# simplify23/MRN

Hardware: AMD Instinct MI355X
Metric: text-line images/sec (fwd+bwd) at 32x256, TRBA+MRN 6 experts (higher is better)
Workload: dtype f32; 1 GPU; MRN loop B: TRBAx6 frozen experts fwd + DM-Router fwd/bwd + clip + Adam, 32x256x4 crops; per_gpu_batch=256, global_batch=256, parallelism=dp1

## Files before the change

mrn_amd/_lib.py:

```python
import ctypes
import os
import re

import torch

_HERE = os.path.dirname(os.path.abspath(__file__))
LIB_PATH = os.environ.get("MRN_LIB_PATH") or os.path.join(_HERE, "csrc", "libmrn_hip.so")
HEADER_PATH = os.path.join(os.path.dirname(_HERE), "include", "mrn_hip.h")
DECODE_HEADER_PATH = os.path.join(os.path.dirname(_HERE), "include", "mrn_decode.h")
ATTN_BEAM_HEADER_PATH = os.path.join(os.path.dirname(_HERE), "include", "mrn_attn_beam.h")
LEXICON_HEADER_PATH = os.path.join(os.path.dirname(_HERE), "include", "mrn_lexicon.h")

_CTYPES = {
    "int": ctypes.c_int,
    "int64_t": ctypes.c_int64,
    "float": ctypes.c_float,
    "void*": ctypes.c_void_p,
    "float*": ctypes.c_void_p,
    "const float*": ctypes.c_void_p,
    "const int64_t*": ctypes.c_void_p,
    "int64_t*": ctypes.c_void_p,
    "const int*": ctypes.c_void_p,
    "int*": ctypes.c_void_p,
    "const int32_t*": ctypes.c_void_p,
    "int32_t*": ctypes.c_void_p,
    "const void*": ctypes.c_void_p,
# ... 24 lines not shown


class _Lib:
    def __init__(self):
        self._dll = None
        self._protos = None

    def load(self):
        if self._dll is not None:
            return self._dll
        if not os.path.exists(LIB_PATH):
            raise RuntimeError(
                f"{LIB_PATH} is missing: build it with `python -m mrn_amd.build` (there is no CPU fallback)")
        dll = ctypes.CDLL(LIB_PATH)
        self._protos = {**parse_header(), **parse_header(DECODE_HEADER_PATH), **parse_header(ATTN_BEAM_HEADER_PATH),
                        **parse_header(LEXICON_HEADER_PATH)}
        for name, (ret, argtypes, _) in self._protos.items():
            fn = getattr(dll, name)
            fn.restype = _CTYPES[ret]
            fn.argtypes = [_CTYPES[t] for t in argtypes]
        self._dll = dll
        return dll

    def call(self, name, *args):
        dll = self.load()
        fn = getattr(dll, name)
        rc = fn(*args)
        if fn.restype is ctypes.c_int and rc != 0:
            msg = dll.mrn_last_error().decode()
            raise RuntimeError(f"{name} failed (code {rc}): {msg}")
        return rc
# ... 8 lines not shown
```

mrn_amd/csrc/common.hpp:

```cpp
#pragma once
#include <hip/hip_runtime.h>
#include <stdint.h>
#include <stdio.h>
#include <string.h>

#define MRN_EXPORT extern "C" __attribute__((visibility("default")))

enum {
  MRN_OK = 0,
  MRN_ERR_BAD_ARG = -1,
  MRN_ERR_UNSUPPORTED = -2,
  MRN_ERR_WORKSPACE = -3,
};

void mrn_set_error(const char* fmt, ...);

#define MRN_CHECK_ARG(cond, ...)          \
  do {                                    \
    if (!(cond)) {                        \
      mrn_set_error(__VA_ARGS__);         \
      return MRN_ERR_BAD_ARG;             \
    }                                     \
  } while (0)

// ... 19 lines not shown
  int base = (xcd < r) ? xcd * (q + 1) : r * (q + 1) + (xcd - r) * q;
  return base + idx;
}

__device__ __forceinline__ void split_f16(float x, _Float16& hi, _Float16& lo) {
  asm volatile("" : "+v"(x));
  hi = (_Float16)x;
  lo = (_Float16)(x - (float)hi);
}

__device__ __forceinline__ void split_f16_sat(float x, _Float16& hi, _Float16& lo) {
  x = fminf(fmaxf(x, -65504.f), 65504.f);
  split_f16(x, hi, lo);
}

__device__ __forceinline__ float relu_nan(float v, float floor_ = 0.f) { return v != v ? v : fmaxf(v, floor_); }
__device__ __forceinline__ float max_nan(float a, float b) { return (a != a || b != b) ? a + b : fmaxf(a, b); }

__device__ __forceinline__ float gelu_fast(float x) {
  const float z = fabsf(x) * 0.70710678118654752440f;
  const float t = __builtin_amdgcn_rcpf(fmaf(0.3275911f, z, 1.f));
  float pl = fmaf(1.061405429f, t, -1.453152027f);
  pl = fmaf(pl, t, 1.421413741f);
  pl = fmaf(pl, t, -0.284496736f);
  pl = fmaf(pl, t, 0.254829592f);
  const float e = pl * t * __builtin_amdgcn_exp2f(-z * z * 1.4426950408889634f);
  const float cdf = x >= 0.f ? fmaf(-0.5f, e, 1.f) : 0.5f * e;
  return x * cdf;
}

// ... 38 lines not shown
```

mrn_amd/csrc/conv_patch.hip:

```cpp
#include "common.hpp"
#include <stdlib.h>

namespace {

typedef _Float16 f16v8 __attribute__((ext_vector_type(8)));
typedef unsigned u32x4 __attribute__((ext_vector_type(4)));
typedef __attribute__((address_space(3))) void* lds_ptr_t;

struct ConvPatchParams {
  const unsigned char* x;
  const unsigned char* w;
  const float* w_scale;
  const float* bias;
  const long long* gamma;
  float* y;
  float* stats;
  long x_gstride;
  int x_bytes;
  int B, H, W, act, pool;
  int tiles_x, tiles_y, tiles;
  int rows;
};

template <int CB, int NCO, int NST>
struct Cfg {
  static constexpr int RG = 4 / NCO;
  static constexpr int TH = 4 * RG, TW = 32;
  static constexpr int PR = TH + 2, PC = TW + 2;
  static constexpr int NL = CB * PR * PC;
  static constexpr int NDMA = (NL + 7) / 8;
  static constexpr int NJ = (NDMA + 3) / 4;
  static constexpr int STAGE = NJ * 4 * 1024;
  static constexpr bool LEAN = CB == 2;
  static constexpr int STATS = LEAN ? 4 * 8 * 64 * 16 : 0;
  static constexpr int LDS = NST * STAGE + STATS;
  static constexpr int NS = CB * 9 * 2;
};

__device__ __forceinline__ f32x16 mma(const u32x4 a, const u32x4 b, const f32x16 c) {
#ifdef MRN_PPROBE_NO_MFMA
  f32x16 r = c;
  r[0] += __builtin_bit_cast(float, a[0] ^ b[0]);
  return r;
#endif
  return __builtin_amdgcn_mfma_f32_32x32x16_f16(*reinterpret_cast<const f16v8*>(&a), *reinterpret_cast<const f16v8*>(&b), c, 0, 0, 0);
}

#ifdef MRN_PPROBE_TIMING
__device__ unsigned long long g_patch_dbg[8];
extern "C" __attribute__((visibility("default"))) int mrn_patch_dbg_read(unsigned long long* out, int reset) {
  if (hipMemcpyFromSymbol(out, HIP_SYMBOL(g_patch_dbg), sizeof(g_patch_dbg)) != hipSuccess) return -1;
  if (reset) {
// ... 1 lines not shown
    (void)hipMemcpyToSymbol(HIP_SYMBOL(g_patch_dbg), z, sizeof(z));
  }
  return 0;
}
#define PTICK(var) const long var = __builtin_readcyclecounter()
#define PADD(slot, a, b) dbg_acc[slot] += (b) - (a)
#else
#define PTICK(var)
#define PADD(slot, a, b)
#endif

__device__ __forceinline__ float swap1(float v) {
  return __builtin_bit_cast(float, __builtin_amdgcn_mov_dpp(__builtin_bit_cast(int, v), 0xB1, 0xF, 0xF, true));
}

template <int CB, int NCO, int NST, bool POOL, int NPROD = 3>
__global__ __launch_bounds__(256) void conv_patch_x3_kernel(const ConvPatchParams p) {
  using C = Cfg<CB, NCO, NST>;
  constexpr int PR = C::PR, PC = C::PC, TH = C::TH, STAGE = C::STAGE;
  extern __shared__ __attribute__((aligned(1024))) unsigned char lds[];
  const int t = threadIdx.x, lane = t & 63, wave = __builtin_amdgcn_readfirstlane(t >> 6);
  const int n = lane & 31, kh = lane >> 5;
  const int g = blockIdx.y;
  const int cob = wave % NCO, rg = wave / NCO;
  const int co0 = cob * 32;
  constexpr int Cout = NCO * 32;

  u32x4 Wh[CB][9][2], Wl[CB][9][2];
  {
    const unsigned char* wg = p.w + ((long)g * Cout + co0 + n) * (CB * 9 * 128) + kh * 16;
#pragma unroll
// ... 36 lines not shown
    a.x0 = (r2 - ty * p.tiles_x) * C::TW;
    a.base = (((a.b * p.H + a.y0 - 1) * p.W + a.x0 - 1) * CB) * 128;
    return a;
  };
  auto issue_dma = [&](int i, const TileAt& a, int stage, bool live) {
    const int L = 8 * (wave + 4 * i) + (lane >> 3);
    const int cb = CB == 1 ? 0 : (L >= PR * PC ? 1 : 0), rem = L - cb * (PR * PC);
    const int prow = (rem * 1928) >> 16, pcol = rem - prow * PC;
    static_assert(PC == 34 && C::NJ * 32 < 1024, "the division by the patch width is a multiply-shift");
    const int y = a.y0 - 1 + prow, x = a.x0 - 1 + pcol;
    const bool ok = live && L < C::NL && (unsigned)y < (unsigned)p.H && (unsigned)x < (unsigned)p.W;
    const int rel = ((prow * p.W + pcol) * CB + cb) * 128 + (((lane & 7) ^ ((pcol >> 1) & 7)) << 4);
    const int okm = -(int)ok;
    const int voff = ((a.base + rel) & okm) | ((int)0x80000000 & ~okm);
    __builtin_amdgcn_raw_ptr_buffer_load_lds(xr, (lds_ptr_t)(lds + stage * STAGE + (wave + 4 * i) * 1024), 16, voff, 0, 0, 0);
  };

  constexpr int RP = 2, NPASS = 4 / RP;
  f32x16 accA[RP], accB[RP];
#pragma unroll
  for (int r = 0; r < RP; ++r)
#pragma unroll
    for (int e = 0; e < 16; ++e) accA[r][e] = accB[r][e] = 0.f;
  f32x4 hold = {0.f, 0.f, 0.f, 0.f};
  struct Pending { int off, ok0, ok1, okp, live; };
  Pending pend = {0, 0, 0, 0, 0};
  constexpr bool LEAN = C::LEAN, PIPE = !LEAN;
  f32x4 st_s[LEAN ? 1 : 4], st_q[LEAN ? 1 : 4];
  f32x4 bias4[LEAN ? 1 : 4];
  unsigned char* const st_base = lds + NST * STAGE + (wave * 8 * 64 + lane) * 16;
// ... 111 lines not shown
      }
      if (LEAN) *reinterpret_cast<f32x4*>(st_base + c * 1024) = f32x4{0.f, 0.f, 0.f, 0.f};
      else if (c < 4) st_s[LEAN ? 0 : c] = f32x4{0.f, 0.f, 0.f, 0.f};
      else st_q[LEAN ? 0 : c - 4] = f32x4{0.f, 0.f, 0.f, 0.f};
    }
    if (n == 0 && p.stats) {
      float* dst = p.stats + (((long)g * p.rows + row) * C::RG + rg) * 2 * Cout + co0 + 4 * kh;
#pragma unroll
      for (int c = 0; c < 8; ++c) *reinterpret_cast<f32x4*>(dst + (c >> 2) * Cout + 8 * (c & 3)) = v[c];
    }
  };
  int row = blockIdx.x, tile = row, stage = 0;
  int flush_row = -1;
  TileAt cur = locate(tile < p.tiles ? tile : 0);
  if (tile < p.tiles) {
#pragma unroll
    for (int i = 0; i < C::NJ; ++i) issue_dma(i, cur, 0, true);
  }
  __builtin_amdgcn_s_waitcnt((7 << 4) | (15 << 8));
#ifdef MRN_PPROBE_TIMING
  long dbg_acc[6] = {0, 0, 0, 0, 0, 0};
#endif
  while (tile < p.tiles) {
    PTICK(tk0);
    asm volatile("s_waitcnt lgkmcnt(0)" ::: "memory");
    __builtin_amdgcn_s_barrier();
    asm volatile("" ::: "memory");
    PTICK(tk1);
    PADD(0, tk0, tk1);
    int nxt = tile + p.rows, nrow = row;
    if (nxt >= p.tiles) {
      nrow = row + gridDim.x;
// ... 16 lines not shown
#pragma unroll
        for (int r = 0; r < RP; ++r) {
          const int imm = (cb * PR + ps * RP + r + dy) * PC * 128;
          if constexpr (NPROD == 3) Xl[set][r] = *reinterpret_cast<const u32x4*>(lds + offv[dx][1][ks] + imm);
          Xh[set][r] = *reinterpret_cast<const u32x4*>(lds + offv[dx][0][ks] + imm);
        }
      };
      PTICK(tm0);
      read_X(0, 0);
      constexpr int DMA_PER_STEP = (C::NJ + C::NS - 3) / (C::NS - 2);
      constexpr int EPI0 = 1;
#pragma unroll
      for (int s = 0; s < C::NS; ++s) {
        const int cb = s / 18, tap = (s % 18) >> 1, ks = s & 1, set = s & 1;
        if (s + 1 < C::NS) read_X(s + 1, set ^ 1);
        if (ps == 0) {
#pragma unroll
          for (int i = s * DMA_PER_STEP; i < (s + 1) * DMA_PER_STEP; ++i)
            if (i < C::NJ) issue_dma(i, nx, stage ^ 1, more);
        }
        if (PIPE && s >= EPI0 && s < EPI0 + 8) epilogue_slice(accp, s - EPI0);
        if constexpr (NPROD == 3) {
#pragma unroll
          for (int r = 0; r < RP; ++r) acc[r] = mma(Wh[cb][tap][ks], Xl[set][r], acc[r]);
#pragma unroll
          for (int r = 0; r < RP; ++r) acc[r] = mma(Wl[cb][tap][ks], Xh[set][r], acc[r]);
        }
#pragma unroll
        for (int r = 0; r < RP; ++r) acc[r] = mma(Wh[cb][tap][ks], Xh[set][r], acc[r]);
#define PATCH_SGB(mask, n) __builtin_amdgcn_sched_group_barrier(mask, n, 0);
#define PATCH_INTERLEAVE PATCH_SGB(0x008, 1) PATCH_SGB(0x002, 6) PATCH_SGB(0x100, 1) PATCH_SGB(0x020, 1) PATCH_SGB(0x040, 1)
        PATCH_INTERLEAVE PATCH_INTERLEAVE
        if constexpr (NPROD == 3) { PATCH_INTERLEAVE PATCH_INTERLEAVE PATCH_INTERLEAVE PATCH_INTERLEAVE }
        __builtin_amdgcn_sched_barrier(0);
      }
      if (ps == 0 && flush_row >= 0) {
        flush_stats(flush_row);
        flush_row = -1;
      }
      pend = make_pending(cur, ps);
      if (!PIPE) {
#pragma unroll
        for (int j = 0; j < 8; ++j) epilogue_slice(acc, j);
        pend.live = 0;
      }
      PTICK(tm1);
      PADD(1, tm0, tm1);
      if (ps == NPASS - 1) __builtin_amdgcn_s_waitcnt((7 << 4) | (15 << 8));
// ... 47 lines not shown

}

MRN_EXPORT int64_t mrn_conv3x3_patch_supported(int Cin, int Cout) { return (Cin == 32 && Cout == 64) || (Cin == 64 && Cout == 128); }

static int patch_rows(long tiles) { return (int)(tiles < 1008 ? tiles : 1008); }

MRN_EXPORT int64_t mrn_conv3x3_patch_stats_blocks(int G, int B, int H, int W, int Cin) {
  (void)G;
  const int TH = Cin == 32 ? 8 : 4, RG = Cin == 32 ? 2 : 1;
  return (int64_t)patch_rows((long)B * ((H + TH - 1) / TH) * ((W + 31) / 32)) * RG;
}

static int patch_launch(const void* x_hl, const void* w_hl, const float* w_scale, const float* bias,
                        const void* bn_gamma_ptrs, float* y, float* stats, int G, int64_t x_group_stride_bytes, int B,
                        int H, int W, int Cin, int Cout, int act, int pool, int products, void* stream) {
  MRN_CHECK_ARG(x_hl && w_hl && w_scale && y && G >= 1 && mrn_conv3x3_patch_supported(Cin, Cout),
                "mrn_conv3x3_patch_x3_hl32: bad operands (Cin=%d Cout=%d)", Cin, Cout);
  MRN_CHECK_ARG(!pool || (H % 2 == 0 && W % 2 == 0), "mrn_conv3x3_patch_x3_hl32: the pooled form needs even H, W (%d x %d)", H, W);
  MRN_CHECK_ARG((long)B * H * W * Cin * 4 < 2147483647L && (long)B * H * W * Cout * 4 < 2147483647L && (uintptr_t)x_hl % 16 == 0 &&
                    (uintptr_t)w_hl % 16 == 0 && (uintptr_t)y % 16 == 0,
                "mrn_conv3x3_patch_x3_hl32: one expert's input and output must stay below 2 GiB each and be 16-byte aligned");
  if (B == 0 || H == 0 || W == 0) return MRN_OK;
  ConvPatchParams p;
  p.x = (const unsigned char*)x_hl; p.w = (const unsigned char*)w_hl; p.w_scale = w_scale; p.bias = bias;
  p.gamma = (const long long*)bn_gamma_ptrs; p.y = y; p.stats = stats; p.x_gstride = x_group_stride_bytes;
  p.x_bytes = (int)((long)B * H * W * Cin * 4);
  p.B = B; p.H = H; p.W = W; p.act = act; p.pool = pool;
  const int TH = Cin == 32 ? 8 : 4;
  p.tiles_x = (W + 31) / 32; p.tiles_y = (H + TH - 1) / TH; p.tiles = B * p.tiles_x * p.tiles_y;
  p.rows = patch_rows(p.tiles);
  int wgs = patch_wgs(G, p.tiles, 1);
  if (wgs > p.rows) wgs = p.rows;
#define PATCH_LAUNCH(CB_, NCO_, POOL_, NP_)                                                                                              \
  do {                                                                                                                                   \
    using C = Cfg<CB_, NCO_, 2>;                                                                                                          \
    static bool set = false;                                                                                                             \
    if (!set) {                                                                                                                          \
      (void)hipFuncSetAttribute((const void*)conv_patch_x3_kernel<CB_, NCO_, 2, POOL_, NP_>, hipFuncAttributeMaxDynamicSharedMemorySize, C::LDS); \
      set = true;                                                                                                                        \
    }                                                                                                                                    \
    hipLaunchKernelGGL((conv_patch_x3_kernel<CB_, NCO_, 2, POOL_, NP_>), dim3(wgs, G), dim3(256), C::LDS, (hipStream_t)stream, p);      \
  } while (0)
#define PATCH_LAUNCH_P(CB_, NCO_, POOL_) do { if (products == 1) PATCH_LAUNCH(CB_, NCO_, POOL_, 1); else PATCH_LAUNCH(CB_, NCO_, POOL_, 3); } while (0)
  if (Cin == 32) {
    if (pool) PATCH_LAUNCH_P(1, 2, true);
    else PATCH_LAUNCH_P(1, 2, false);
  } else {
    if (pool) PATCH_LAUNCH_P(2, 4, true);
    else PATCH_LAUNCH_P(2, 4, false);
  }
#undef PATCH_LAUNCH_P
#undef PATCH_LAUNCH
  MRN_LAUNCH_CHECK("conv3x3_patch_x3");
  return MRN_OK;
}

MRN_EXPORT int mrn_conv3x3_patch_x3_hl32(const void* x_hl, const void* w_hl, const float* w_scale, const float* bias,
                                         const void* bn_gamma_ptrs, float* y, float* stats, int G, int64_t x_group_stride_bytes, int B,
                                         int H, int W, int Cin, int Cout, int act, int pool, void* stream) {
  return patch_launch(x_hl, w_hl, w_scale, bias, bn_gamma_ptrs, y, stats, G, x_group_stride_bytes, B, H, W, Cin, Cout, act, pool, 3, stream);
}

MRN_EXPORT int mrn_conv3x3_patch_x1_hl32(const void* x_hl, const void* w_hl, const float* w_scale, const float* bias,
                                         const void* bn_gamma_ptrs, float* y, float* stats, int G, int64_t x_group_stride_bytes, int B,
                                         int H, int W, int Cin, int Cout, int act, int pool, void* stream) {
  return patch_launch(x_hl, w_hl, w_scale, bias, bn_gamma_ptrs, y, stats, G, x_group_stride_bytes, B, H, W, Cin, Cout, act, pool, 1, stream);
}
```

mrn_amd/csrc/group_ops.hip:

```cpp
#include "common.hpp"

namespace {

typedef _Float16 f16v8 __attribute__((ext_vector_type(8)));
typedef _Float16 f16v4 __attribute__((ext_vector_type(4)));

struct F8 {
  f32x4 a, b;
};

__device__ __forceinline__ F8 load8(const float* p) {
  F8 v;
  v.a = *reinterpret_cast<const f32x4*>(p);
  v.b = *reinterpret_cast<const f32x4*>(p + 4);
  return v;
}
__device__ __forceinline__ void store8(float* p, const F8& v) {
  *reinterpret_cast<f32x4*>(p) = v.a;
  *reinterpret_cast<f32x4*>(p + 4) = v.b;
}
__device__ __forceinline__ void store_hl(unsigned char* out, long row, int C, int c8, const F8& v) {
  f16v8 h, l;
#pragma unroll
  for (int e = 0; e < 4; ++e) {
    _Float16 hh, ll;
    split_f16_sat(v.a[e], hh, ll);
    h[e] = hh; l[e] = ll;
    split_f16_sat(v.b[e], hh, ll);
    h[4 + e] = hh; l[4 + e] = ll;
  }
  unsigned char* o = out + (row * (C >> 5) + (c8 >> 2)) * 128 + (c8 & 3) * 16;
  *reinterpret_cast<f16v8*>(o) = h;
  *reinterpret_cast<f16v8*>(o + 64) = l;
}

__device__ __forceinline__ void store_d16(unsigned char* out, long row, int C, int c8, const F8& v, int dense = 1) {
  unsigned char* dst = out + (row * (C >> 6) + (c8 >> 3)) * 128 + (c8 & 7) * 16;
  if (dense == 2) {
    typedef unsigned short u16v8 __attribute__((ext_vector_type(8)));
    u16v8 h;
#pragma unroll
    for (int e = 0; e < 8; ++e) {
      const unsigned u = __float_as_uint(e < 4 ? v.a[e] : v.b[e - 4]);
      h[e] = (unsigned short)((u + 0x7fffu + ((u >> 16) & 1u)) >> 16);
    }
// ... 793 lines not shown
```

mrn_amd/modules/expert_group.py:

```python
import os

import torch

from .. import ops
from ._nn import _pair, packed_weight, require_no_grad, to_nhwc
from .geometry import check_call, geometry_supported, unsupported_geometry_message


EVAL_BN_FOLD = os.environ.get("MRN_EVAL_BN_FOLD", "1") != "0"
SVTR_GROUPED_EMBED = os.environ.get("MRN_SVTR_EMBED", "grouped") == "grouped"
TPS_WINO = os.environ.get("MRN_TPS_WINO", "1") == "1"
EVAL_WINO = os.environ.get("MRN_EVAL_WINO", "1") != "0"
SHORTCUT_BN_FOLD = os.environ.get("MRN_SHORTCUT_BN_FOLD", "1") != "0"
RESIDUAL_FROM_F32 = bool(int(os.environ.get("MRN_RESIDUAL_F32", "0")))


def conv_out_rows(H, pool):
    return H if pool is None else ops.conv_out_hw(H, 1, pool[0], pool[1], pool[2])[0]


class Act:

    def __init__(self, shape, f32=None, hl=None, shared=False, wino=None, wino_R=0, affine=None):
        self.shape = tuple(shape)
# ... 95 lines not shown
        key = tuple(t.data_ptr() for b in bns for t in (b.weight, b.bias, b.running_mean, b.running_var))
        got = self._bncache.get(id(bns[0]))
        if got is None or got[0] != key:
            rows = [[b.weight.data_ptr() for b in bns], [b.bias.data_ptr() for b in bns],
                    [b.running_mean.data_ptr() for b in bns], [b.running_var.data_ptr() for b in bns]]
            got = (key, torch.tensor(rows, dtype=torch.int64, device=bns[0].weight.device))
            self._bncache[id(bns[0])] = got
        return got[1]

    def _bias_stack(self, convs):
        if convs[0].bias is None:
            return None
        return torch.stack([c.bias.detach() for c in convs]).contiguous()

    def layer(self, x, convs, bns=None, relu=True, residual=None, pool=None, want_f32=False, want_hl=True, want_wino=0, gelu=False,
              height_mean=False, defer_affine=False):
        if defer_affine and (bns is None or relu or pool is not None or want_hl or want_wino or height_mean or gelu or residual is not None
                             or not want_f32):
            raise ValueError("layer(defer_affine=True) takes a BatchNorm layer with relu=False, want_f32=True and no pool, want_hl, "
                             "want_wino, height_mean, gelu or residual")
        if gelu:
            assert bns is not None and bns[0].training and pool is None and not want_wino and residual is None
            relu = True
        G = self.G
        _, B, H, W, Cin = x.shape
        c0 = convs[0]
        Cout = c0.out_channels
        ksize, stride, padding = _pair(c0.kernel_size), _pair(c0.stride), _pair(c0.padding)
        Ho, Wo = ops.conv_out_hw(H, W, ksize, stride, padding)
        dev = c0.weight.device
        training = bns is not None and bns[0].training
# ... 1 lines not shown
        act = ops.ACT_RELU if (fuse_act and relu) else ops.ACT_NONE
        stats = None
        res = residual.f32 if residual is not None else None
        res_hl = residual.hl if residual is not None and res is None else None
        res_affine = residual.affine if residual is not None else None
        use_wino = x.wino is not None and x.wino_R == self.wino_for(c0, bns, H)
        if want_wino and not ops.wino_rows_fit(conv_out_rows(Ho, pool)):
            want_wino, want_hl = 0, True
        height_mean = height_mean and Ho > 1 and self._height_mean
        if height_mean:
            assert pool is None and residual is None and not want_wino and not gelu
        patch_pool = (pool == ((2, 2), (2, 2), (0, 0)) and Ho % 2 == 0 and Wo % 2 == 0
                      and ops.patch_conv_supported(ksize, stride, padding, Cin, Cout))
        eval_fold = (EVAL_BN_FOLD and bns is not None and not training and Cin % 32 == 0 and Cout >= 64 and Cout % 32 == 0
                     and (want_hl or res_hl is None) and not use_wino and not want_wino and not patch_pool and not height_mean)
        if res_affine is not None and (eval_fold or pool is not None or height_mean):
            ops.bn_apply_grouped(res, res_affine[0], res_affine[1], relu=False, want_f32=True, want_hl=False)
            residual.affine = res_affine = None
        if eval_fold:
            if x.hl is None:
                assert x.f32 is not None
                x.hl = ops.split_hl32(x.f32)
            w_hl, w_scale = self._weights_hl(convs)
            scale, shift = ops.bn_eval_affine_grouped(self._bn_table(bns), G, Cout, bns[0].eps)
            fused = dict(bias=self._bias_stack(convs), act=ops.ACT_RELU if relu else ops.ACT_NONE, ch_scale=scale, ch_shift=shift,
                         residual=res, residual_hl=res_hl, products=ops.X3_PRODUCTS)
            if pool is not None:
                assert res is None and res_hl is None
                y, _ = ops.conv2d_x3(x.hl, G, x.shared, B, H, W, Cin, w_hl, w_scale, Cout, ksize, stride, padding, **fused)
                f32, hl, (Hp, Wp) = ops.maxpool_grouped(y, pool[0], pool[1], pool[2], None, None, relu=False, want_f32=want_f32,
                                                        want_hl=want_hl)
                return Act((G, B, Hp, Wp, Cout), f32, hl)
            got, _ = ops.conv2d_x3(x.hl, G, x.shared, B, H, W, Cin, w_hl, w_scale, Cout, ksize, stride, padding,
                                   hl_only=want_hl and not want_f32, also_hl=want_hl and want_f32, **fused)
            if want_hl and want_f32:
                return Act((G, B, Ho, Wo, Cout), got[0], got[1])
            return Act((G, B, Ho, Wo, Cout), None, got) if want_hl else Act((G, B, Ho, Wo, Cout), got, None)
        use_patch = not use_wino and (x.hl is not None or x.f32 is not None) and ops.patch_conv_supported(ksize, stride, padding, Cin, Cout)
        use_c4 = (not use_patch and not use_wino and Cin == 4 and ksize == (3, 3) and stride == (1, 1) and padding == (1, 1)
                  and Cout in (32, 64) and x.f32 is not None)
        pooled = ((use_patch or (use_c4 and ops.PATCH_CONV) or (use_wino and ops.wino_pool_supported(H, W, x.wino_R, Cout)))
                  and pool == ((2, 2), (2, 2), (0, 0)) and Ho % 2 == 0 and Wo % 2 == 0)
        y = torch.empty(G, B, Ho // 2 if pooled else Ho, Wo // 2 if pooled else Wo, Cout, device=dev, dtype=torch.float32)
        if use_patch:
            if x.hl is None:
                x.hl = ops.split_hl32(x.f32)
            w_hl, w_scale = self._weights_hl(convs)
            _, stats = ops.conv3x3_patch_x3(x.hl, G, x.shared, B, H, W, Cin, w_hl, w_scale, Cout, bias=self._bias_stack(convs), act=act,
                                            want_stats=training, pool=pooled, gamma_ptrs=self._bn_table(bns)[0] if bns is not None else None,
                                            out=y)
            if pooled:
                pool = None
        elif use_wino:
            u_hl, u_scale = self._weights_wino(convs, x.wino_R)
            _, stats = ops.conv2d_x3_wino(x.wino, G, x.shared, B, H, W, Cin, u_hl, u_scale, Cout, x.wino_R,
                                          bias=self._bias_stack(convs), act=act, want_stats=training, out=y, pool=pooled,
                                          gamma_ptrs=self._bn_table(bns)[0] if (pooled and bns is not None) else None)
            if pooled:
                pool = None
        elif Cin % 32 == 0 and Cout >= 64:
            if x.hl is None:
                assert x.f32 is not None
                x.hl = ops.split_hl32(x.f32)
            w_hl, w_scale = self._weights_hl(convs)
            _, stats = ops.conv2d_x3(x.hl, G, x.shared, B, H, W, Cin, w_hl, w_scale, Cout, ksize, stride, padding,
# ... 27 lines not shown
            if want_wino:
                f32, hl, v, (Hp, Wp) = ops.maxpool_wino_grouped(y, pool[0], pool[1], pool[2], want_wino, scale, shift, relu=post_relu,
                                                                want_f32=want_f32, want_hl=want_hl)
                return Act((G, B, Hp, Wp, Cout), f32, hl, wino=v, wino_R=want_wino)
            f32, hl, (Hp, Wp) = ops.maxpool_grouped(y, pool[0], pool[1], pool[2], scale, shift, relu=post_relu,
                                                    want_f32=want_f32, want_hl=want_hl)
            return Act((G, B, Hp, Wp, Cout), f32, hl)
        Ho, Wo = y.shape[2], y.shape[3]
        if height_mean:
            f32, hl = ops.height_mean_grouped(y, scale, shift, relu=post_relu, want_f32=want_f32, want_hl=want_hl)
            return Act((G, B, 1, Wo, Cout), None if f32 is None else f32.view(G, B, 1, Wo, Cout), hl)
        if scale is None and res is None and res_hl is None and not post_relu and not want_hl and not want_wino:
            return Act((G, B, Ho, Wo, Cout), y, None)
        if defer_affine:
            return Act((G, B, Ho, Wo, Cout), y, None, affine=(scale, shift))
        if want_wino:
            f32, hl, v = ops.bn_apply_wino_grouped(y, scale, shift, want_wino, relu=post_relu, residual=res, residual_hl=res_hl,
                                                   want_f32=want_f32, want_hl=want_hl, residual_affine=res_affine)
            return Act((G, B, Ho, Wo, Cout), f32, hl, wino=v, wino_R=want_wino)
        f32, hl = ops.bn_apply_grouped(y, scale, shift, relu=2 if (gelu and post_relu) else post_relu, residual=res, want_f32=want_f32,
                                       want_hl=want_hl, residual_hl=res_hl, residual_affine=res_affine)
        return Act((G, B, Ho, Wo, Cout), f32, hl)

    def _basic_block(self, x, blocks, next_needs_f32, out_wino=0, out_hl=True):
        b0 = blocks[0]
        w2 = self.wino_for(b0.conv2, [b.bn2 for b in blocks])
        out = self.layer(x, [b.conv1 for b in blocks], [b.bn1 for b in blocks], want_wino=w2, want_hl=not w2)
        if b0.downsample is not None:
            res = self.layer(x, [b.downsample[0] for b in blocks], [b.downsample[1] for b in blocks], relu=False,
                             want_f32=True, want_hl=False, defer_affine=SHORTCUT_BN_FOLD)
        else:
            res = x
            assert res.f32 is not None or res.hl is not None
        return self.layer(out, [b.conv2 for b in blocks], [b.bn2 for b in blocks], relu=True, residual=res,
                          want_f32=next_needs_f32, want_hl=out_hl, want_wino=out_wino)

    def _batched_linear_f32(self, name, x, layers, act=ops.ACT_NONE):
# ... 20 lines not shown
                    ow, oh = self.wino_for(nxt[0].conv1, [b.bn1 for b in nxt]), True
                else:
                    ow = self.wino_for(getattr(n0, after), [getattr(n, after_bn) for n in nets])
                    oh = not ow
                x = self._basic_block(x, [b[i] for b in blocks], RESIDUAL_FROM_F32 and i + 1 < nb and blocks[0][i + 1].downsample is None,
                                      out_wino=ow, out_hl=oh)
            return x

        def first_wino(name):
            blk = [getattr(n, name)[0] for n in nets]
            return self.wino_for(blk[0].conv1, [b.bn1 for b in blk])

        def first_block_identity(name):
            return RESIDUAL_FROM_F32 and getattr(n0, name)[0].downsample is None

        x = self.layer(x, [n.conv0_1 for n in nets], [n.bn0_1 for n in nets])
        x = self.layer(x, [n.conv0_2 for n in nets], [n.bn0_2 for n in nets], pool=p22, want_f32=first_block_identity("layer1"))
        x = stage(x, "layer1", "conv1", "bn1")
        x = self.layer(x, [n.conv1 for n in nets], [n.bn1 for n in nets], pool=p22, want_f32=first_block_identity("layer2"),
                       want_wino=first_wino("layer2"))
        x = stage(x, "layer2", "conv2", "bn2")
        x = self.layer(x, [n.conv2 for n in nets], [n.bn2 for n in nets], pool=p2_21, want_f32=first_block_identity("layer3"),
                       want_wino=first_wino("layer3"))
        x = stage(x, "layer3", "conv3", "bn3")
        x = self.layer(x, [n.conv3 for n in nets], [n.bn3 for n in nets], want_f32=first_block_identity("layer4"),
                       want_wino=first_wino("layer4"))
        x = stage(x, "layer4", "conv4_1", "bn4_1")
        x = self.layer(x, [n.conv4_1 for n in nets], [n.bn4_1 for n in nets])
        return self.layer(x, [n.conv4_2 for n in nets], [n.bn4_2 for n in nets], want_f32=not last_hl, want_hl=last_hl, height_mean=True)

    def _vgg(self, x, last_hl=False):
# ... 168 lines not shown
            N = H * W
            gm, bt = self._ln_params("svtr_sub%d" % si, [s.norm for s in subs])
            last = si == 2
            _, x, hl = ops.add_layernorm_grouped(y.f32.view(G * B, N, C), None, None, N, gm, bt, B * N, subs[0].norm.eps,
                                                 want_f32=not (last and last_hl), want_hl=last and last_hl)
        return Act((G, B, H, W, C), x.view(G, B, H, W, C) if x is not None else None, hl if last_hl else None)

    def _tps(self, image):
        G = self.G
        B, H, W, C = image.shape
        tps = [e.Transformation for e in self.experts]
        loc = [t.LocalizationNetwork for t in tps]
        pool = ((2, 2), (2, 2), (0, 0))
        x = Act((G, B, H, W, C), image, None, shared=True)
        w2, w3, w4 = (self.wino_for(loc[0].conv[i], [l.conv[i + 1] for l in loc]) if TPS_WINO else 0 for i in (4, 8, 12))
        x = self.layer(x, [l.conv[0] for l in loc], [l.conv[1] for l in loc], pool=pool, want_wino=w2, want_hl=not w2)
        x = self.layer(x, [l.conv[4] for l in loc], [l.conv[5] for l in loc], pool=pool, want_wino=w3, want_hl=not w3)
        x = self.layer(x, [l.conv[8] for l in loc], [l.conv[9] for l in loc], pool=pool, want_wino=w4, want_hl=not w4)
        x = self.layer(x, [l.conv[12] for l in loc], [l.conv[13] for l in loc], want_f32=True, want_hl=False)
        out = torch.empty(G, B, tps[0].I_r_size[0], tps[0].I_r_size[1], C, device=image.device, dtype=torch.float32)
        _, _, Hl, Wl, Cl = x.shape
        v = ops.avgpool_nhwc(x.f32.view(G * B, Hl, Wl, Cl))
        fc1s, fc2s = [l.localization_fc1[0] for l in loc], [l.localization_fc2 for l in loc]
        v = self._batched_linear_f32("loc_fc1", v.view(G, B, Cl), fc1s, act=ops.ACT_RELU)
        cp = self._batched_linear_f32("loc_fc2", v, fc2s).view(G, B, loc[0].F, 2)
        for g, t in enumerate(tps):
            gg = t.GridGenerator
            ops.tps_grid_sample(image, cp[g], gg.inv_delta_C, gg.P_hat, t.I_r_size, out=out[g])
        return Act(tuple(out.shape), out, None)

    def visual_all(self, image, as_act=False):
# ... 161 lines not shown
```

mrn_amd/ops.py:

```python
import os
import sys
import weakref

import torch

from ._lib import call
from .modules.label_length import ctc_label_length_supported, ctc_uses_long_kernel, unsupported_label_length_message
from .modules.task_count import router_uses_wide_kernels, tasks_supported, unsupported_task_count_message

ACT_NONE, ACT_RELU, ACT_GELU = 0, 1, 2


class KernelTimer:

    def __init__(self, only=None):
        self.spans = []
        self.only = only

    def begin(self, site="other"):
        if self.only is not None and site not in self.only:
            return None
        e = torch.cuda.Event(enable_timing=True)
        e.record()
        return e
# ... 852 lines not shown
         Cout, act, int(bool(pool)), _p(gamma_ptrs), _stream())
    if t0 is not None:
        CONV_TIMER.end(t0, 2.0 * G * B * H * W * Cout * 36, ("f32mfma/" if pool else "hbm/") + "conv_first_kernel<%d%s>" % (Cout // 32, ", true" if pool else ""),
                       4.0 * ((1 if shared else G) * B * H * W * 4 + G * B * Ho * Wo * Cout))
    return y, stats


PATCH_CONV = os.environ.get("MRN_PATCH_CONV", "1") == "1"


def patch_conv_supported(ksize, stride, padding, Cin, Cout):
    return (PATCH_CONV and tuple(ksize) == (3, 3) and tuple(stride) == (1, 1) and tuple(padding) == (1, 1)
            and bool(call("mrn_conv3x3_patch_supported", Cin, Cout)))


def conv3x3_patch_x3(x_hl, G, shared_input, B, H, W, Cin, w_hl, w_scale, Cout, bias=None, act=ACT_NONE, want_stats=False, pool=False,
                     gamma_ptrs=None, out=None):
    dev = x_hl.device
    Ho, Wo = (H // 2, W // 2) if pool else (H, W)
    y = out if out is not None else torch.empty(G, B, Ho, Wo, Cout, device=dev, dtype=torch.float32)
    stats = None
    if want_stats:
        stats = torch.empty(G, call("mrn_conv3x3_patch_stats_blocks", G, B, H, W, Cin), 2, Cout, device=dev, dtype=torch.float32)
    timed = CONV_TIMER is not None
    t0 = CONV_TIMER.begin() if timed else None
    one = X3_PRODUCTS == 1
    call("mrn_conv3x3_patch_x1_hl32" if one else "mrn_conv3x3_patch_x3_hl32", _p(x_hl), _p(w_hl), _p(w_scale), _p(bias), _p(gamma_ptrs), _p(y),
         _p(stats), G, 0 if shared_input else B * H * W * Cin * 4, B, H, W, Cin, Cout, act, int(bool(pool)), _stream())
    if timed:
        nbytes = 4.0 * ((1 if shared_input else G) * B * H * W * Cin + G * Cout * 9 * Cin + G * B * Ho * Wo * Cout)
        kind = ("fp16" if one else "fp16x3") + "/patch%d" % Cin + ("pool" if pool else "")
        if TIMER_SHAPES:
            kind += "|G%d B%d %dx%d %d->%d k3x3 s11" % (G, B, H, W, Cin, Cout)
        CONV_TIMER.end(t0, 2.0 * G * B * H * W * Cout * 9 * Cin, kind, nbytes)
    return y, stats


_FINALIZE_TICKETS = {}


def _finalize_tickets(device, slots):
    key = _dev_stream()
    t = _FINALIZE_TICKETS.get(key)
    if t is None or t.numel() < slots:
        t = torch.zeros(max(slots, 1024), device=device, dtype=torch.int32)
        _FINALIZE_TICKETS[key] = t
# ... 1526 lines not shown
```

Baseline: 3144 images/s.

## Fuse BatchNorm apply and hi/lo fp16 split into patch conv input load

Adds an f32-input variant of the split-fp16 patch conv kernel that loads raw fp32 activations, applies the previous layer's BatchNorm scale/shift and ReLU, splits to hi/lo fp16 and writes to LDS. The loads and conversions are spread across the MFMA steps of the previous tile. Two layers (conv0_1 in the feature extractor, the first TPS localization conv) now return deferred-affine outputs for this reader. This removes a separate bn_apply pass and its hl buffer round trip through HBM. In exchange it uses more registers, LDS and VALU work inside the conv main loop, which could hurt MFMA throughput.

```diff
diff --git a/include/mrn_conv_patch.h b/include/mrn_conv_patch.h
--- /dev/null
+++ b/include/mrn_conv_patch.h
@@ -0,0 +1,16 @@
+#ifndef MRN_CONV_PATCH_H
+#define MRN_CONV_PATCH_H
+#include <stdint.h>
+
+#ifdef __cplusplus
+extern "C" {
+#endif
+
+int mrn_conv3x3_patch_x3_f32in(const float* x_f32, const float* in_scale, const float* in_shift, int in_relu, const void* w_hl,
+                               const float* w_scale, const float* bias, const void* bn_gamma_ptrs, float* y, float* stats, int G,
+                               int64_t x_group_stride_bytes, int B, int H, int W, int Cin, int Cout, int act, int pool, void* stream);
+
+#ifdef __cplusplus
+}
+#endif
+#endif
diff --git a/mrn_amd/_lib.py b/mrn_amd/_lib.py
--- a/mrn_amd/_lib.py
+++ b/mrn_amd/_lib.py
@@ -10,6 +10,7 @@
 DECODE_HEADER_PATH = os.path.join(os.path.dirname(_HERE), "include", "mrn_decode.h")
 ATTN_BEAM_HEADER_PATH = os.path.join(os.path.dirname(_HERE), "include", "mrn_attn_beam.h")
 LEXICON_HEADER_PATH = os.path.join(os.path.dirname(_HERE), "include", "mrn_lexicon.h")
+CONV_PATCH_HEADER_PATH = os.path.join(os.path.dirname(_HERE), "include", "mrn_conv_patch.h")
 
 _CTYPES = {
     "int": ctypes.c_int,
@@ -64,7 +65,7 @@
                 f"{LIB_PATH} is missing: build it with `python -m mrn_amd.build` (there is no CPU fallback)")
         dll = ctypes.CDLL(LIB_PATH)
         self._protos = {**parse_header(), **parse_header(DECODE_HEADER_PATH), **parse_header(ATTN_BEAM_HEADER_PATH),
-                        **parse_header(LEXICON_HEADER_PATH)}
+                        **parse_header(LEXICON_HEADER_PATH), **parse_header(CONV_PATCH_HEADER_PATH)}
         for name, (ret, argtypes, _) in self._protos.items():
             fn = getattr(dll, name)
             fn.restype = _CTYPES[ret]
diff --git a/mrn_amd/csrc/common.hpp b/mrn_amd/csrc/common.hpp
--- a/mrn_amd/csrc/common.hpp
+++ b/mrn_amd/csrc/common.hpp
@@ -57,6 +57,17 @@
   split_f16(x, hi, lo);
 }
 
+typedef _Float16 f16x8 __attribute__((ext_vector_type(8)));
+__device__ __forceinline__ void split_hl4(const f32x4 v, int e0, f16x8& h, f16x8& l) {
+#pragma unroll
+  for (int e = 0; e < 4; ++e) {
+    _Float16 hh, ll;
+    split_f16_sat(v[e], hh, ll);
+    h[e0 + e] = hh;
+    l[e0 + e] = ll;
+  }
+}
+
 __device__ __forceinline__ float relu_nan(float v, float floor_ = 0.f) { return v != v ? v : fmaxf(v, floor_); }
 __device__ __forceinline__ float max_nan(float a, float b) { return (a != a || b != b) ? a + b : fmaxf(a, b); }
 
diff --git a/mrn_amd/csrc/conv_patch.hip b/mrn_amd/csrc/conv_patch.hip
--- a/mrn_amd/csrc/conv_patch.hip
+++ b/mrn_amd/csrc/conv_patch.hip
@@ -20,6 +20,9 @@
   int B, H, W, act, pool;
   int tiles_x, tiles_y, tiles;
   int rows;
+  const float* in_scale;
+  const float* in_shift;
+  int in_relu;
 };
 
 template <int CB, int NCO, int NST>
@@ -35,7 +38,23 @@
   static constexpr int STATS = LEAN ? 4 * 8 * 64 * 16 : 0;
   static constexpr int LDS = NST * STAGE + STATS;
   static constexpr int NS = CB * 9 * 2;
+  static constexpr int NU = (PR * PC * 4 + 255) / 256;
+  static constexpr int NK = CB * NU;
 };
+
+template <bool PIPE, int NS, int NK>
+constexpr int load_unit_at(int ps, int s) {
+  const int gs = ps * NS + s;
+  if (PIPE) return gs < NK ? gs : -1;
+  return (gs % 7 == 0 && gs / 7 < NK) ? gs / 7 : -1;
+}
+template <bool PIPE, int NS, int NK>
+constexpr int cvt_slice_at(int ps, int s) {
+  static_assert(PIPE ? (NS == 18 && NK * 3 == 18) : (7 * (NK - 1) + 14 < 2 * NS), "every conversion slice has its step");
+  if (PIPE) return s >= 9 ? ps * 9 + (s - 9) : -1;
+  const int d = ps * NS + s - 10, k = d / 7, r = d % 7;
+  return (d >= 0 && k < NK && r < 5 && !(r & 1)) ? 3 * k + r / 2 : -1;
+}
 
 __device__ __forceinline__ f32x16 mma(const u32x4 a, const u32x4 b, const f32x16 c) {
 #ifdef MRN_PPROBE_NO_MFMA
@@ -67,7 +86,7 @@
   return __builtin_bit_cast(float, __builtin_amdgcn_mov_dpp(__builtin_bit_cast(int, v), 0xB1, 0xF, 0xF, true));
 }
 
-template <int CB, int NCO, int NST, bool POOL, int NPROD = 3>
+template <int CB, int NCO, int NST, bool POOL, int NPROD = 3, bool F32IN = false>
 __global__ __launch_bounds__(256) void conv_patch_x3_kernel(const ConvPatchParams p) {
   using C = Cfg<CB, NCO, NST>;
   constexpr int PR = C::PR, PC = C::PC, TH = C::TH, STAGE = C::STAGE;
@@ -134,6 +153,81 @@
     const int okm = -(int)ok;
     const int voff = ((a.base + rel) & okm) | ((int)0x80000000 & ~okm);
     __builtin_amdgcn_raw_ptr_buffer_load_lds(xr, (lds_ptr_t)(lds + stage * STAGE + (wave + 4 * i) * 1024), 16, voff, 0, 0, 0);
+  };
+
+  constexpr int NU = F32IN ? C::NU : 1, NK = F32IN ? C::NK : 1;
+  constexpr bool HOLD = !C::LEAN;
+  static_assert(64 * C::NU + 63 < 1024 && C::NU <= 32, "multiply-shift division; one validity bit per unit");
+  struct Unit { int prow, pcol, rel, ldo; };
+  auto unit_geom = [&](int i) {
+    Unit u;
+    const int j = t & 3, l0 = (t >> 2) + 64 * i, line = l0 < PR * PC ? l0 : PR * PC - 1;
+    u.prow = (line * 1928) >> 16;
+    u.pcol = line - u.prow * PC;
+    u.rel = (u.prow * p.W + u.pcol) * (CB * 128) + j * 32;
+    u.ldo = line * 128 + ((j ^ ((u.pcol >> 1) & 7)) << 4);
+    return u;
+  };
+  Unit u_held[HOLD ? NU : 1];
+  unsigned char* const aff = lds + C::LDS;
+  if constexpr (F32IN) {
+    if (HOLD) {
+#pragma unroll
+      for (int i = 0; i < NU; ++i) u_held[HOLD ? i : 0] = unit_geom(i);
+    }
+    if (t < CB * 32) {
+      reinterpret_cast<float*>(aff)[t] = p.in_scale[(long)g * (CB * 32) + t];
+      reinterpret_cast<float*>(aff)[CB * 32 + t] = p.in_shift[(long)g * (CB * 32) + t];
+    }
+    __syncthreads();
+  }
+  auto unit_of = [&](int i) { return HOLD ? u_held[HOLD ? i : 0] : unit_geom(i); };
+  const float in_floor = p.in_relu ? 0.f : -INFINITY;
+  f32x4 raw[NK][2];
+  unsigned u_ok = 0;
+  f16x8 cvt_h, cvt_l;
+  auto issue_load = [&](int k, const TileAt& a, bool live) {
+    const int cb = k / NU, i = k % NU;
+    const Unit u = unit_of(i);
+    if (cb == 0) {
+      const int y = a.y0 - 1 + u.prow, x = a.x0 - 1 + u.pcol;
+      const unsigned ok = (unsigned)live & (unsigned)((unsigned)y < (unsigned)p.H) & (unsigned)((unsigned)x < (unsigned)p.W);
+      u_ok = (u_ok & ~(1u << i)) | (ok << i);
+    }
+    const int okm = -(int)((u_ok >> i) & 1u);
+    const int voff = ((a.base + u.rel) & okm) | ((int)0x80000000 & ~okm);
+#pragma unroll
+    for (int h = 0; h < 2; ++h)
+      raw[k][h] = __builtin_bit_cast(f32x4, __builtin_amdgcn_raw_buffer_load_b128(xr, voff + cb * 128 + h * 16, 0, 0));
+  };
+  auto convert_slice = [&](int k, int part, int wbase) {
+    const int cb = k / NU, i = k % NU;
+    if (part == 0) {
+#pragma unroll
+      for (int h = 0; h < 2; ++h) {
+        const f32x4 sc = *reinterpret_cast<const f32x4*>(aff + (cb * 32 + (t & 3) * 8 + h * 4) * 4);
+        const f32x4 sh = *reinterpret_cast<const f32x4*>(aff + (CB * 32 + cb * 32 + (t & 3) * 8 + h * 4) * 4);
+#pragma unroll
+        for (int e = 0; e < 4; ++e) {
+          const float v = raw[k][h][e] * sc[e] + sh[e];
+          raw[k][h][e] = relu_nan(v, in_floor);
+        }
+      }
+    } else if (part == 1) {
+      split_hl4(raw[k][0], 0, cvt_h, cvt_l);
+    } else {
+      split_hl4(raw[k][1], 4, cvt_h, cvt_l);
+      const unsigned okm = -((u_ok >> i) & 1u);
+      u32x4 hb = __builtin_bit_cast(u32x4, cvt_h), lb = __builtin_bit_cast(u32x4, cvt_l);
+#pragma unroll
+      for (int e = 0; e < 4; ++e) {
+        hb[e] &= okm;
+        lb[e] &= okm;
+      }
+      const int wo = wbase + cb * (PR * PC * 128) + unit_of(i).ldo;
+      *reinterpret_cast<u32x4*>(lds + wo) = hb;
+      *reinterpret_cast<u32x4*>(lds + (wo ^ 64)) = lb;
+    }
   };
 
   constexpr int RP = 2, NPASS = 4 / RP;
@@ -275,8 +369,17 @@
   int flush_row = -1;
   TileAt cur = locate(tile < p.tiles ? tile : 0);
   if (tile < p.tiles) {
-#pragma unroll
-    for (int i = 0; i < C::NJ; ++i) issue_dma(i, cur, 0, true);
+    if constexpr (F32IN) {
+#pragma unroll
+      for (int k = 0; k < NK; ++k) {
+        issue_load(k, cur, true);
+#pragma unroll
+        for (int part = 0; part < 3; ++part) convert_slice(k, part, 0);
+      }
+    } else {
+#pragma unroll
+      for (int i = 0; i < C::NJ; ++i) issue_dma(i, cur, 0, true);
+    }
   }
   __builtin_amdgcn_s_waitcnt((7 << 4) | (15 << 8));
 #ifdef MRN_PPROBE_TIMING
@@ -323,7 +426,12 @@
       for (int s = 0; s < C::NS; ++s) {
         const int cb = s / 18, tap = (s % 18) >> 1, ks = s & 1, set = s & 1;
         if (s + 1 < C::NS) read_X(s + 1, set ^ 1);
-        if (ps == 0) {
+        if constexpr (F32IN) {
+          const int lu = load_unit_at<PIPE, C::NS, NK>(ps, s);
+          if (lu >= 0) issue_load(lu, nx, more);
+          const int sl = cvt_slice_at<PIPE, C::NS, NK>(ps, s);
+          if (sl >= 0) convert_slice(sl / 3, sl % 3, (stage ^ 1) * STAGE);
+        } else if (ps == 0) {
 #pragma unroll
           for (int i = s * DMA_PER_STEP; i < (s + 1) * DMA_PER_STEP; ++i)
             if (i < C::NJ) issue_dma(i, nx, stage ^ 1, more);
@@ -339,8 +447,13 @@
         for (int r = 0; r < RP; ++r) acc[r] = mma(Wh[cb][tap][ks], Xh[set][r], acc[r]);
 #define PATCH_SGB(mask, n) __builtin_amdgcn_sched_group_barrier(mask, n, 0);
 #define PATCH_INTERLEAVE PATCH_SGB(0x008, 1) PATCH_SGB(0x002, 6) PATCH_SGB(0x100, 1) PATCH_SGB(0x020, 1) PATCH_SGB(0x040, 1)
-        PATCH_INTERLEAVE PATCH_INTERLEAVE
-        if constexpr (NPROD == 3) { PATCH_INTERLEAVE PATCH_INTERLEAVE PATCH_INTERLEAVE PATCH_INTERLEAVE }
+#define PATCH_INTERLEAVE_W PATCH_SGB(0x008, 1) PATCH_SGB(0x002, 6) PATCH_SGB(0x100, 1) PATCH_SGB(0x200, 1) PATCH_SGB(0x020, 1) PATCH_SGB(0x040, 1)
+        if constexpr (F32IN) {
+          PATCH_INTERLEAVE_W PATCH_INTERLEAVE_W PATCH_INTERLEAVE_W PATCH_INTERLEAVE_W PATCH_INTERLEAVE_W PATCH_INTERLEAVE_W
+        } else {
+          PATCH_INTERLEAVE PATCH_INTERLEAVE
+          if constexpr (NPROD == 3) { PATCH_INTERLEAVE PATCH_INTERLEAVE PATCH_INTERLEAVE PATCH_INTERLEAVE }
+        }
         __builtin_amdgcn_sched_barrier(0);
       }
       if (ps == 0 && flush_row >= 0) {
@@ -418,7 +531,8 @@
 
 static int patch_launch(const void* x_hl, const void* w_hl, const float* w_scale, const float* bias,
                         const void* bn_gamma_ptrs, float* y, float* stats, int G, int64_t x_group_stride_bytes, int B,
-                        int H, int W, int Cin, int Cout, int act, int pool, int products, void* stream) {
+                        int H, int W, int Cin, int Cout, int act, int pool, int products, void* stream,
+                        const float* in_scale = nullptr, const float* in_shift = nullptr, int in_relu = 0) {
   MRN_CHECK_ARG(x_hl && w_hl && w_scale && y && G >= 1 && mrn_conv3x3_patch_supported(Cin, Cout),
                 "mrn_conv3x3_patch_x3_hl32: bad operands (Cin=%d Cout=%d)", Cin, Cout);
   MRN_CHECK_ARG(!pool || (H % 2 == 0 && W % 2 == 0), "mrn_conv3x3_patch_x3_hl32: the pooled form needs even H, W (%d x %d)", H, W);
@@ -431,22 +545,29 @@
   p.gamma = (const long long*)bn_gamma_ptrs; p.y = y; p.stats = stats; p.x_gstride = x_group_stride_bytes;
   p.x_bytes = (int)((long)B * H * W * Cin * 4);
   p.B = B; p.H = H; p.W = W; p.act = act; p.pool = pool;
+  p.in_scale = in_scale; p.in_shift = in_shift; p.in_relu = in_relu;
   const int TH = Cin == 32 ? 8 : 4;
   p.tiles_x = (W + 31) / 32; p.tiles_y = (H + TH - 1) / TH; p.tiles = B * p.tiles_x * p.tiles_y;
   p.rows = patch_rows(p.tiles);
   int wgs = patch_wgs(G, p.tiles, 1);
   if (wgs > p.rows) wgs = p.rows;
-#define PATCH_LAUNCH(CB_, NCO_, POOL_, NP_)                                                                                              \
+  const int aff_bytes = in_scale ? 512 : 0;
+#define PATCH_LAUNCH(CB_, NCO_, POOL_, NP_, ...)                                                                                         \
   do {                                                                                                                                   \
     using C = Cfg<CB_, NCO_, 2>;                                                                                                          \
     static bool set = false;                                                                                                             \
     if (!set) {                                                                                                                          \
-      (void)hipFuncSetAttribute((const void*)conv_patch_x3_kernel<CB_, NCO_, 2, POOL_, NP_>, hipFuncAttributeMaxDynamicSharedMemorySize, C::LDS); \
+      (void)hipFuncSetAttribute((const void*)conv_patch_x3_kernel<CB_, NCO_, 2, POOL_, NP_, ##__VA_ARGS__>, hipFuncAttributeMaxDynamicSharedMemorySize, C::LDS + 512); \
       set = true;                                                                                                                        \
     }                                                                                                                                    \
-    hipLaunchKernelGGL((conv_patch_x3_kernel<CB_, NCO_, 2, POOL_, NP_>), dim3(wgs, G), dim3(256), C::LDS, (hipStream_t)stream, p);      \
+    hipLaunchKernelGGL((conv_patch_x3_kernel<CB_, NCO_, 2, POOL_, NP_, ##__VA_ARGS__>), dim3(wgs, G), dim3(256), C::LDS + aff_bytes, (hipStream_t)stream, p); \
   } while (0)
-#define PATCH_LAUNCH_P(CB_, NCO_, POOL_) do { if (products == 1) PATCH_LAUNCH(CB_, NCO_, POOL_, 1); else PATCH_LAUNCH(CB_, NCO_, POOL_, 3); } while (0)
+#define PATCH_LAUNCH_P(CB_, NCO_, POOL_)                      \
+  do {                                                        \
+    if (in_scale) PATCH_LAUNCH(CB_, NCO_, POOL_, 3, true);    \
+    else if (products == 1) PATCH_LAUNCH(CB_, NCO_, POOL_, 1); \
+    else PATCH_LAUNCH(CB_, NCO_, POOL_, 3);                   \
+  } while (0)
   if (Cin == 32) {
     if (pool) PATCH_LAUNCH_P(1, 2, true);
     else PATCH_LAUNCH_P(1, 2, false);
@@ -471,3 +592,13 @@
                                          int H, int W, int Cin, int Cout, int act, int pool, void* stream) {
   return patch_launch(x_hl, w_hl, w_scale, bias, bn_gamma_ptrs, y, stats, G, x_group_stride_bytes, B, H, W, Cin, Cout, act, pool, 1, stream);
 }
+
+MRN_EXPORT int mrn_conv3x3_patch_x3_f32in(const float* x_f32, const float* in_scale, const float* in_shift, int in_relu, const void* w_hl,
+                                          const float* w_scale, const float* bias, const void* bn_gamma_ptrs, float* y, float* stats, int G,
+                                          int64_t x_group_stride_bytes, int B, int H, int W, int Cin, int Cout, int act, int pool,
+                                          void* stream) {
+  MRN_CHECK_ARG(in_scale && in_shift && (uintptr_t)in_scale % 16 == 0 && (uintptr_t)in_shift % 16 == 0,
+                "mrn_conv3x3_patch_x3_f32in: in_scale / in_shift [G][Cin] are required, 16-byte aligned");
+  return patch_launch(x_f32, w_hl, w_scale, bias, bn_gamma_ptrs, y, stats, G, x_group_stride_bytes, B, H, W, Cin, Cout, act, pool, 3, stream,
+                      in_scale, in_shift, in_relu != 0);
+}
diff --git a/mrn_amd/csrc/group_ops.hip b/mrn_amd/csrc/group_ops.hip
--- a/mrn_amd/csrc/group_ops.hip
+++ b/mrn_amd/csrc/group_ops.hip
@@ -21,14 +21,8 @@
 }
 __device__ __forceinline__ void store_hl(unsigned char* out, long row, int C, int c8, const F8& v) {
   f16v8 h, l;
-#pragma unroll
-  for (int e = 0; e < 4; ++e) {
-    _Float16 hh, ll;
-    split_f16_sat(v.a[e], hh, ll);
-    h[e] = hh; l[e] = ll;
-    split_f16_sat(v.b[e], hh, ll);
-    h[4 + e] = hh; l[4 + e] = ll;
-  }
+  split_hl4(v.a, 0, h, l);
+  split_hl4(v.b, 4, h, l);
   unsigned char* o = out + (row * (C >> 5) + (c8 >> 2)) * 128 + (c8 & 3) * 16;
   *reinterpret_cast<f16v8*>(o) = h;
   *reinterpret_cast<f16v8*>(o + 64) = l;
diff --git a/mrn_amd/modules/expert_group.py b/mrn_amd/modules/expert_group.py
--- a/mrn_amd/modules/expert_group.py
+++ b/mrn_amd/modules/expert_group.py
@@ -133,7 +133,7 @@
         return torch.stack([c.bias.detach() for c in convs]).contiguous()
 
     def layer(self, x, convs, bns=None, relu=True, residual=None, pool=None, want_f32=False, want_hl=True, want_wino=0, gelu=False,
-              height_mean=False, defer_affine=False):
+              height_mean=False, defer_affine=False, raw_for_patch=False):
         if defer_affine and (bns is None or relu or pool is not None or want_hl or want_wino or height_mean or gelu or residual is not None
                              or not want_f32):
             raise ValueError("layer(defer_affine=True) takes a BatchNorm layer with relu=False, want_f32=True and no pool, want_hl, "
@@ -165,6 +165,10 @@
                       and ops.patch_conv_supported(ksize, stride, padding, Cin, Cout))
         eval_fold = (EVAL_BN_FOLD and bns is not None and not training and Cin % 32 == 0 and Cout >= 64 and Cout % 32 == 0
                      and (want_hl or res_hl is None) and not use_wino and not want_wino and not patch_pool and not height_mean)
+        patch_in = ops.patch_conv_supported(ksize, stride, padding, Cin, Cout) and not use_wino
+        if x.affine is not None and not (len(x.affine) == 3 and patch_in and not eval_fold and ops.patch_bn_on_load(Cin)):
+            _, x.hl = ops.bn_apply_grouped(x.f32, x.affine[0], x.affine[1], relu=x.affine[2], want_f32=False, want_hl=True)
+            x.f32 = x.affine = None
         if res_affine is not None and (eval_fold or pool is not None or height_mean):
             ops.bn_apply_grouped(res, res_affine[0], res_affine[1], relu=False, want_f32=True, want_hl=False)
             residual.affine = res_affine = None
@@ -194,12 +198,12 @@
                   and pool == ((2, 2), (2, 2), (0, 0)) and Ho % 2 == 0 and Wo % 2 == 0)
         y = torch.empty(G, B, Ho // 2 if pooled else Ho, Wo // 2 if pooled else Wo, Cout, device=dev, dtype=torch.float32)
         if use_patch:
-            if x.hl is None:
+            if x.affine is None and x.hl is None:
                 x.hl = ops.split_hl32(x.f32)
             w_hl, w_scale = self._weights_hl(convs)
-            _, stats = ops.conv3x3_patch_x3(x.hl, G, x.shared, B, H, W, Cin, w_hl, w_scale, Cout, bias=self._bias_stack(convs), act=act,
-                                            want_stats=training, pool=pooled, gamma_ptrs=self._bn_table(bns)[0] if bns is not None else None,
-                                            out=y)
+            _, stats = ops.conv3x3_patch_x3(x.hl if x.affine is None else x.f32, G, x.shared, B, H, W, Cin, w_hl, w_scale, Cout,
+                                            bias=self._bias_stack(convs), act=act, want_stats=training, pool=pooled,
+                                            gamma_ptrs=self._bn_table(bns)[0] if bns is not None else None, out=y, in_affine=x.affine)
             if pooled:
                 pool = None
         elif use_wino:
@@ -257,6 +261,9 @@
             return Act((G, B, Ho, Wo, Cout), y, None)
         if defer_affine:
             return Act((G, B, Ho, Wo, Cout), y, None, affine=(scale, shift))
+        if (raw_for_patch and scale is not None and res is None and res_hl is None and want_hl and not want_f32 and not want_wino
+                and not gelu):
+            return Act((G, B, Ho, Wo, Cout), y, None, affine=(scale, shift, post_relu))
         if want_wino:
             f32, hl, v = ops.bn_apply_wino_grouped(y, scale, shift, want_wino, relu=post_relu, residual=res, residual_hl=res_hl,
                                                    want_f32=want_f32, want_hl=want_hl, residual_affine=res_affine)
@@ -264,6 +271,11 @@
         f32, hl = ops.bn_apply_grouped(y, scale, shift, relu=2 if (gelu and post_relu) else post_relu, residual=res, want_f32=want_f32,
                                        want_hl=want_hl, residual_hl=res_hl, residual_affine=res_affine)
         return Act((G, B, Ho, Wo, Cout), f32, hl)
+
+    @staticmethod
+    def patch_reader(conv):
+        return (ops.patch_conv_supported(_pair(conv.kernel_size), _pair(conv.stride), _pair(conv.padding), conv.in_channels,
+                                         conv.out_channels) and ops.patch_bn_on_load(conv.in_channels))
 
     def _basic_block(self, x, blocks, next_needs_f32, out_wino=0, out_hl=True):
         b0 = blocks[0]
@@ -314,7 +326,7 @@
         def first_block_identity(name):
             return RESIDUAL_FROM_F32 and getattr(n0, name)[0].downsample is None
 
-        x = self.layer(x, [n.conv0_1 for n in nets], [n.bn0_1 for n in nets])
+        x = self.layer(x, [n.conv0_1 for n in nets], [n.bn0_1 for n in nets], raw_for_patch=self.patch_reader(n0.conv0_2))
         x = self.layer(x, [n.conv0_2 for n in nets], [n.bn0_2 for n in nets], pool=p22, want_f32=first_block_identity("layer1"))
         x = stage(x, "layer1", "conv1", "bn1")
         x = self.layer(x, [n.conv1 for n in nets], [n.bn1 for n in nets], pool=p22, want_f32=first_block_identity("layer2"),
@@ -513,7 +525,8 @@
         pool = ((2, 2), (2, 2), (0, 0))
         x = Act((G, B, H, W, C), image, None, shared=True)
         w2, w3, w4 = (self.wino_for(loc[0].conv[i], [l.conv[i + 1] for l in loc]) if TPS_WINO else 0 for i in (4, 8, 12))
-        x = self.layer(x, [l.conv[0] for l in loc], [l.conv[1] for l in loc], pool=pool, want_wino=w2, want_hl=not w2)
+        x = self.layer(x, [l.conv[0] for l in loc], [l.conv[1] for l in loc], pool=pool, want_wino=w2, want_hl=not w2,
+                       raw_for_patch=self.patch_reader(loc[0].conv[4]))
         x = self.layer(x, [l.conv[4] for l in loc], [l.conv[5] for l in loc], pool=pool, want_wino=w3, want_hl=not w3)
         x = self.layer(x, [l.conv[8] for l in loc], [l.conv[9] for l in loc], pool=pool, want_wino=w4, want_hl=not w4)
         x = self.layer(x, [l.conv[12] for l in loc], [l.conv[13] for l in loc], want_f32=True, want_hl=False)
diff --git a/mrn_amd/ops.py b/mrn_amd/ops.py
--- a/mrn_amd/ops.py
+++ b/mrn_amd/ops.py
@@ -890,8 +890,18 @@
             and bool(call("mrn_conv3x3_patch_supported", Cin, Cout)))
 
 
+PATCH_BN_ON_LOAD = os.environ.get("MRN_PATCH_BN_ON_LOAD", "1")
+
+
+def patch_bn_on_load(Cin):
+    return X3_PRODUCTS == 3 and PATCH_BN_ON_LOAD in ("1", str(Cin))
+
+
 def conv3x3_patch_x3(x_hl, G, shared_input, B, H, W, Cin, w_hl, w_scale, Cout, bias=None, act=ACT_NONE, want_stats=False, pool=False,
-                     gamma_ptrs=None, out=None):
+                     gamma_ptrs=None, out=None, in_affine=None):
+    if in_affine is not None:
+        return _conv3x3_patch_x3_f32in(x_hl, in_affine, G, shared_input, B, H, W, Cin, w_hl, w_scale, Cout, bias, act, want_stats, pool,
+                                       gamma_ptrs, out)
     dev = x_hl.device
     Ho, Wo = (H // 2, W // 2) if pool else (H, W)
     y = out if out is not None else torch.empty(G, B, Ho, Wo, Cout, device=dev, dtype=torch.float32)
@@ -906,6 +916,33 @@
     if timed:
         nbytes = 4.0 * ((1 if shared_input else G) * B * H * W * Cin + G * Cout * 9 * Cin + G * B * Ho * Wo * Cout)
         kind = ("fp16" if one else "fp16x3") + "/patch%d" % Cin + ("pool" if pool else "")
+        if TIMER_SHAPES:
+            kind += "|G%d B%d %dx%d %d->%d k3x3 s11" % (G, B, H, W, Cin, Cout)
+        CONV_TIMER.end(t0, 2.0 * G * B * H * W * Cout * 9 * Cin, kind, nbytes)
+    return y, stats
+
+
+def _conv3x3_patch_x3_f32in(x_f32, in_affine, G, shared_input, B, H, W, Cin, w_hl, w_scale, Cout, bias, act, want_stats, pool, gamma_ptrs,
+                            out):
+    scale, shift, relu = in_affine
+    if X3_PRODUCTS != 3:
+        raise RuntimeError("conv3x3_patch_x3(in_affine=...) exists for the split-fp16 x3 products only")
+    if (x_f32.dtype != torch.float32 or not x_f32.is_contiguous() or x_f32.numel() != (1 if shared_input else G) * B * H * W * Cin
+            or tuple(scale.shape) != (G, Cin) or tuple(shift.shape) != (G, Cin) or not scale.is_contiguous() or not shift.is_contiguous()):
+        raise ValueError("conv3x3_patch_x3(in_affine=...): x must be the contiguous fp32 map [G or 1,B,H,W,Cin], scale / shift [G,Cin]")
+    dev = x_f32.device
+    Ho, Wo = (H // 2, W // 2) if pool else (H, W)
+    y = out if out is not None else torch.empty(G, B, Ho, Wo, Cout, device=dev, dtype=torch.float32)
+    stats = None
+    if want_stats:
+        stats = torch.empty(G, call("mrn_conv3x3_patch_stats_blocks", G, B, H, W, Cin), 2, Cout, device=dev, dtype=torch.float32)
+    timed = CONV_TIMER is not None
+    t0 = CONV_TIMER.begin() if timed else None
+    call("mrn_conv3x3_patch_x3_f32in", _p(x_f32), _p(scale), _p(shift), int(bool(relu)), _p(w_hl), _p(w_scale), _p(bias), _p(gamma_ptrs),
+         _p(y), _p(stats), G, 0 if shared_input else B * H * W * Cin * 4, B, H, W, Cin, Cout, act, int(bool(pool)), _stream())
+    if timed:
+        nbytes = 4.0 * ((1 if shared_input else G) * B * H * W * Cin + G * Cout * 9 * Cin + G * B * Ho * Wo * Cout)
+        kind = "fp16x3/patch%d" % Cin + ("pool" if pool else "")
         if TIMER_SHAPES:
             kind += "|G%d B%d %dx%d %d->%d k3x3 s11" % (G, B, H, W, Cin, Cout)
         CONV_TIMER.end(t0, 2.0 * G * B * H * W * Cout * 9 * Cin, kind, nbytes)
```

Result: no change. 3165 images/s, median of 6 (+0.7%).
